# JasonHopeSpace/panda

Measured on AMD Instinct MI355X. Metric: MSM points/s (BN254, 2^24), higher is better.
Workload: dtype u32; 1 GPU; BN254 MSM 2^24 points per GPU, Jacobian output, bases and scalars resident in HBM; curve=bn254, log_points_per_gpu=24, exchange=none

## Files before the change

### panda_amd/csrc/msm_sort.hip

```cpp
#include <algorithm>
#include <atomic>
#include <cmath>

#include "fe29.h"
#include "msm_sort.h"

using namespace panda29;

namespace {

constexpr unsigned SORT_TILE = 8192;
constexpr unsigned MAX_PARTS = 1024;
constexpr unsigned SORT_THREADS = 1024;
constexpr unsigned BS_CHUNK = 8192;

template <class Code>
struct CodeTraits;
template <>
struct CodeTraits<uint16_t> {
    static constexpr u32 ZERO = 0x7fffu;
    static constexpr u32 MAG = 0x7fffu;
    static constexpr int SIGN = 15;
};
template <>
struct CodeTraits<u32> {
    static constexpr u32 ZERO = 0x7fffffffu;
    static constexpr u32 MAG = 0x7fffffffu;
    static constexpr int SIGN = 31;
};

template <int WORDS>
__device__ __forceinline__ void load_words(u32 *dst, const u32 *src)
{
    static_assert(WORDS % 4 == 0, "vector loads");
    const uint4 *s4 = reinterpret_cast<const uint4 *>(src);
#pragma unroll
    for (int i = 0; i < WORDS / 4; i++) {
        uint4 v = s4[i];
        dst[4 * i] = v.x;
        dst[4 * i + 1] = v.y;
        dst[4 * i + 2] = v.z;
        dst[4 * i + 3] = v.w;
    }
}

__device__ __forceinline__ void check_samples(const panda::SampleCheck &sc)
{
    int differs = 0;
    for (unsigned t = threadIdx.x >> 2; t < panda::REG_SAMPLES; t += blockDim.x >> 2) {
        const u64 row = panda::sample_row(t, sc.n);
        for (unsigned k = threadIdx.x & 3u; k < sc.row_words; k += 4) differs |= sc.samples[t * sc.row_words + k] != sc.wire[row * sc.row_words + k];
    }
    differs = __syncthreads_or(differs);
    if (threadIdx.x == 0) {
        *sc.flag_dev = differs ? 1u : 0u;
        if (differs) *sc.flag_host = 1u;
    }
}

struct DigitsBatch {
    unsigned log_n, prefix_bit;
};

template <class Fr, class Code, bool BATCH = false>
__global__ void __launch_bounds__(256) k_digits(const u32 *__restrict__ scalars, Code *__restrict__ dig, u64 n, panda::WindowPlan plan, panda::SampleCheck sc,
                                                DigitsBatch bg)
{
    typedef CodeTraits<Code> CT;
    constexpr int L = Fr::L;
    if (blockIdx.x == 0 && sc.wire) check_samples(sc);
    u64 i = (u64)blockIdx.x * blockDim.x + threadIdx.x;
    if (i >= n) return;
    u32 w[L], s[L + 1];
    load_words<L>(w, scalars + i * L);
    fe_wire_to_canonical<Fr>(s, w);
    s[L] = 0;
    u32 carry = 0;
    const u32 prefix = BATCH ? (u32)(i >> bg.log_n) << bg.prefix_bit : 0u;
    for (unsigned k = 0; k < plan.W; k++) {
        const unsigned c = plan.width[k];
        const u32 half = 1u << (c - 1), full = 1u << c, mask = full - 1;
        unsigned lo = plan.lo[k], m = lo >> 5, sh = lo & 31;
        u32 raw = 0;
        if (m < (unsigned)L) {
            u64 v = s[m] | ((u64)s[m + 1] << 32);
            raw = (u32)(v >> sh) & mask;
        }
        raw += carry;
        u32 code;
        if (raw >= half) {
            u32 mag = full - raw;
            carry = 1;
            code = mag ? ((1u << CT::SIGN) | prefix | (mag - 1)) : CT::ZERO;
        } else {
            carry = 0;
            code = raw ? (prefix | (raw - 1)) : CT::ZERO;
        }
        dig[(u64)k * n + i] = (Code)code;
    }
}

struct DigitsHistGeom {
    unsigned lo_bits, H, tiles;
};

template <class Fr, class Code, bool BATCH = false>
__global__ void __launch_bounds__(1024) k_digits_hist(const u32 *__restrict__ scalars, Code *__restrict__ dig, u32 *__restrict__ tile_hist, u64 n,
                                                     panda::WindowPlan plan, DigitsHistGeom g, panda::SampleCheck sc, DigitsBatch bg)
{
    typedef CodeTraits<Code> CT;
    constexpr int L = Fr::L;
    extern __shared__ u32 hist[];
    if (blockIdx.x == 0 && sc.wire) check_samples(sc);
    const unsigned tile = blockIdx.x, tid = threadIdx.x;
    const unsigned WH = plan.W * g.H, threads = blockDim.x;
    for (unsigned i = tid; i < WH; i += threads) hist[i] = 0;
    __syncthreads();
    const u64 begin = (u64)tile * SORT_TILE, end = begin + SORT_TILE < n ? begin + SORT_TILE : n;
    for (u64 i = begin + tid; i < end; i += threads) {
        u32 w[L], s[L + 1];
        load_words<L>(w, scalars + i * L);
        fe_wire_to_canonical<Fr>(s, w);
        s[L] = 0;
        u32 carry = 0;
        const u32 prefix = BATCH ? (u32)(i >> bg.log_n) << bg.prefix_bit : 0u;
        for (unsigned k = 0; k < plan.W; k++) {
            const unsigned c = plan.width[k];
            const u32 half = 1u << (c - 1), full = 1u << c, mask = full - 1;
            unsigned lo = plan.lo[k], m = lo >> 5, sh = lo & 31;
            u32 raw = 0;
            if (m < (unsigned)L) {
                u64 v = s[m] | ((u64)s[m + 1] << 32);
                raw = (u32)(v >> sh) & mask;
            }
            raw += carry;
            u32 code;
            if (raw >= half) {
                u32 mag = full - raw;
                carry = 1;
                code = mag ? ((1u << CT::SIGN) | prefix | (mag - 1)) : CT::ZERO;
            } else {
                carry = 0;
                code = raw ? (prefix | (raw - 1)) : CT::ZERO;
            }
            dig[(u64)k * n + i] = (Code)code;
            if (code != CT::ZERO) atomicAdd(&hist[k * g.H + ((code & CT::MAG) >> g.lo_bits)], 1u);
        }
    }
    __syncthreads();
    for (unsigned i = tid; i < WH; i += threads) {
        const unsigned k = i / g.H, h = i - k * g.H;
        tile_hist[((u64)k * g.tiles + tile) * g.H + h] = hist[i];
    }
}

template <class Code, class Fn>
__device__ __forceinline__ void for_each_code(const Code *__restrict__ dw, u64 begin, u64 end, Fn f)
{
    constexpr unsigned PER = 16 / sizeof(Code);
    if (reinterpret_cast<uintptr_t>(dw + begin) & 15) {
        for (u64 a = begin + threadIdx.x; a < end; a += blockDim.x) f(a, (u32)dw[a]);
        return;
    }
    for (u64 a = begin + (u64)threadIdx.x * PER; a < end; a += (u64)blockDim.x * PER) {
        const uint4 v = *reinterpret_cast<const uint4 *>(dw + a);
        const u32 wv[4] = {v.x, v.y, v.z, v.w};
#pragma unroll
        for (unsigned j = 0; j < PER; j++) {
            const u32 code = sizeof(Code) == 2 ? (wv[j >> 1] >> (16 * (j & 1))) & 0xffffu : wv[j];
            if (a + j < end) f(a + j, code);
        }
    }
}


struct SortGeom {
    unsigned log_n, lo_bits, H, tiles;
    u32 row0;
};

template <class Code>
__global__ void __launch_bounds__(256) k_part_hist(const Code *__restrict__ dig, u32 *__restrict__ tile_hist, SortGeom g)
{
    typedef CodeTraits<Code> CT;
    __shared__ u32 h[MAX_PARTS];
    const unsigned w = blockIdx.y, tile = blockIdx.x, tid = threadIdx.x;
    for (unsigned i = tid; i < g.H; i += 256) h[i] = 0;
    __syncthreads();
    const u64 n = (u64)1 << g.log_n;
    const Code *dw = dig + ((u64)w << g.log_n);
    const u64 begin = (u64)tile * SORT_TILE, end = begin + SORT_TILE < n ? begin + SORT_TILE : n;
    for_each_code<Code>(dw, begin, end, [&](u64, u32 code) {
        if (code != CT::ZERO) atomicAdd(&h[(code & CT::MAG) >> g.lo_bits], 1u);
    });
    __syncthreads();
    u32 *out = tile_hist + ((u64)w * g.tiles + tile) * g.H;
    for (unsigned i = tid; i < g.H; i += 256) out[i] = h[i];
}

__global__ void __launch_bounds__(1024) k_part_scan_cols(const u32 *__restrict__ tile_hist, u32 *__restrict__ tile_pref, u32 *__restrict__ totals, SortGeom g)
{
    const unsigned w = blockIdx.y, lane = threadIdx.x & 63, h = blockIdx.x * 16 + (threadIdx.x >> 6);
    if (h >= g.H) return;
    const u64 col = (u64)w * g.tiles * g.H + h;
    u32 run = 0;
    for (unsigned t0 = 0; t0 < g.tiles; t0 += 64) {
        const unsigned tile = t0 + lane;
        u32 v = tile < g.tiles ? tile_hist[col + (u64)tile * g.H] : 0;
        u32 inc = v;
        for (unsigned d = 1; d < 64; d <<= 1) {
            u32 up = __shfl_up(inc, d, 64);
            if (lane >= d) inc += up;
        }
        if (tile < g.tiles) tile_pref[col + (u64)tile * g.H] = run + inc - v;
        run += __shfl(inc, 63, 64);
    }
    if (lane == 0) totals[(u64)w * g.H + h] = run;
}

__global__ void __launch_bounds__(1024) k_part_offsets(const u32 *__restrict__ totals, u32 *__restrict__ part_off, SortGeom g)
{
    __shared__ u32 tot[MAX_PARTS];
    const unsigned w = blockIdx.x, t = threadIdx.x;
    const u32 mine = t < g.H ? totals[(u64)w * g.H + t] : 0;
    tot[t] = mine;
    __syncthreads();
    for (unsigned d = 1; d < 1024; d <<= 1) {
        u32 v = (t >= d) ? tot[t - d] : 0;
        __syncthreads();
        tot[t] += v;
        __syncthreads();
    }
    if (t < g.H) part_off[(u64)w * (g.H + 1) + t] = tot[t] - mine;
    if (t == 1023) part_off[(u64)w * (g.H + 1) + g.H] = tot[1023];
}

template <unsigned THREADS = SORT_THREADS>
__device__ __forceinline__ void block_exclusive_scan(u32 *a, unsigned count, u32 *scratch )
{
    const unsigned tid = threadIdx.x;
    const unsigned per = (count + THREADS - 1) / THREADS;
    u32 local = 0;
    for (unsigned j = 0; j < per; j++) {
        unsigned i = tid * per + j;
        if (i < count) local += a[i];
    }
    scratch[tid] = local;
    __syncthreads();
    for (unsigned d = 1; d < THREADS; d <<= 1) {
        u32 v = (tid >= d) ? scratch[tid - d] : 0;
        __syncthreads();
        scratch[tid] += v;
        __syncthreads();
    }
    u32 run = scratch[tid] - local;
    for (unsigned j = 0; j < per; j++) {
        unsigned i = tid * per + j;
        if (i < count) {
            u32 v = a[i];
            a[i] = run;
            run += v;
        }
    }
    __syncthreads();
}

template <class Code, class Word>
__global__ void __launch_bounds__(SORT_THREADS) k_part_scatter(const Code *__restrict__ dig, const u32 *__restrict__ tile_hist, const u32 *__restrict__ tile_pref,
                                                      const u32 *__restrict__ part_off, Word *__restrict__ p1, SortGeom g)
{
    typedef CodeTraits<Code> CT;
    __shared__ u32 lstart[MAX_PARTS];
    __shared__ u32 lcur[MAX_PARTS];
    __shared__ u32 gbase[MAX_PARTS];
    __shared__ Word words[SORT_TILE];
    __shared__ uint16_t parts_of[SORT_TILE];
    __shared__ u32 scratch[SORT_THREADS];
    const unsigned w = blockIdx.y, tile = blockIdx.x, tid = threadIdx.x;
    const u64 row = ((u64)w * g.tiles + tile) * g.H;
    const u32 *po = part_off + (u64)w * (g.H + 1);
    for (unsigned i = tid; i < g.H; i += SORT_THREADS) {
        lstart[i] = tile_hist[row + i];
        lcur[i] = 0;
        gbase[i] = po[i] + tile_pref[row + i];
    }
    __syncthreads();
    const u64 n = (u64)1 << g.log_n;
    const Code *dw = dig + ((u64)w << g.log_n);
    Word *pw = p1 + ((u64)w << g.log_n);
    const u64 begin = (u64)tile * SORT_TILE, end = begin + SORT_TILE < n ? begin + SORT_TILE : n;
    const u32 lo_mask = (1u << g.lo_bits) - 1;
    block_exclusive_scan(lstart, g.H, scratch);
    for_each_code<Code>(dw, begin, end, [&](u64 i, u32 code) {
        if (code == CT::ZERO) return;
        u32 b = code & CT::MAG, h = b >> g.lo_bits;
        u32 slot = lstart[h] + atomicAdd(&lcur[h], 1u);
        words[slot] = ((Word)(b & lo_mask) << (g.log_n + 1)) | (Word)(((code >> CT::SIGN) << g.log_n) | (u32)i);
        parts_of[slot] = (uint16_t)h;
    });
    __syncthreads();
    const u32 total = lstart[g.H - 1] + lcur[g.H - 1];
    for (u32 j = tid; j < total; j += SORT_THREADS) {
        u32 h = parts_of[j];
        pw[gbase[h] + (j - lstart[h])] = words[j];
    }
}

template <class Code>
__global__ void __launch_bounds__(SORT_THREADS) k1_scatter_split(const Code *__restrict__ dig, const u32 *__restrict__ tile_hist, const u32 *__restrict__ tile_pref,
                                                        const u32 *__restrict__ part_off, u32 *__restrict__ p1_lo, unsigned char *__restrict__ p1_hi, SortGeom g,
                                                        unsigned b3)
{
    typedef CodeTraits<Code> CT;
    __shared__ u32 lstart[MAX_PARTS];
    __shared__ u32 lcur[MAX_PARTS];
    __shared__ u32 gbase[MAX_PARTS];
    __shared__ u32 words[SORT_TILE];
    __shared__ unsigned char his[SORT_TILE];
    __shared__ uint16_t parts_of[SORT_TILE];
    __shared__ u32 scratch[SORT_THREADS];
    const unsigned w = blockIdx.y, tile = blockIdx.x, tid = threadIdx.x;
    const u64 row = ((u64)w * g.tiles + tile) * g.H;
    const u32 *po = part_off + (u64)w * (g.H + 1);
    for (unsigned i = tid; i < g.H; i += SORT_THREADS) {
        lstart[i] = tile_hist[row + i];
        lcur[i] = 0;
        gbase[i] = po[i] + tile_pref[row + i];
    }
    __syncthreads();
    const u64 n = (u64)1 << g.log_n;
    const Code *dw = dig + ((u64)w << g.log_n);
    u32 *plo = p1_lo + ((u64)w << g.log_n);
    unsigned char *phi = p1_hi + ((u64)w << g.log_n);
    const u64 begin = (u64)tile * SORT_TILE, end = begin + SORT_TILE < n ? begin + SORT_TILE : n;
    const u32 b3_mask = (1u << b3) - 1, b2_mask = (1u << (g.lo_bits - b3)) - 1;
    block_exclusive_scan(lstart, g.H, scratch);
    for_each_code<Code>(dw, begin, end, [&](u64 i, u32 code) {
        if (code == CT::ZERO) return;
        u32 b = code & CT::MAG, h = b >> g.lo_bits;
        u32 slot = lstart[h] + atomicAdd(&lcur[h], 1u);
        words[slot] = ((b & b3_mask) << (g.log_n + 1)) | ((code >> CT::SIGN) << g.log_n) | (u32)i;
        his[slot] = (unsigned char)((b >> b3) & b2_mask);
        parts_of[slot] = (uint16_t)h;
    });
    __syncthreads();
    const u32 total = lstart[g.H - 1] + lcur[g.H - 1];
    for (u32 j = tid; j < total; j += SORT_THREADS) {
        const u32 h = parts_of[j];
        const u32 dst = gbase[h] + (j - lstart[h]);
        plo[dst] = words[j];
        phi[dst] = his[j];
    }
}

__device__ __forceinline__ void scan128_inclusive(u32 *cnt, u32 *carry )
{
    const unsigned tid = threadIdx.x, lane = tid & 63u;
    u32 v = tid < 128 ? cnt[tid] : 0;
    if (tid < 128) {
        for (unsigned d = 1; d < 64; d <<= 1) {
            const u32 up = __shfl_up(v, d, 64);
            if (lane >= d) v += up;
        }
        if (tid == 63) *carry = v;
    }
    __syncthreads();
    if (tid >= 64 && tid < 128) v += *carry;
    if (tid < 128) cnt[tid] = v;
    __syncthreads();
}

__global__ void __launch_bounds__(SORT_THREADS) k_bucket_sort(const u32 *__restrict__ p1, const u32 *__restrict__ part_off, u32 *__restrict__ off,
                                                     u32 *__restrict__ sorted, SortGeom g, unsigned NB)
{
    __shared__ u32 cnt[128], cur[128], lstart[128], lcur[128], scan_carry;
    __shared__ u32 words[BS_CHUNK];
    __shared__ unsigned char lo_of[BS_CHUNK];
    const unsigned w = blockIdx.y, h = blockIdx.x, tid = threadIdx.x;
    const unsigned L = 1u << g.lo_bits;
    const u32 ps = part_off[(u64)w * (g.H + 1) + h], pe = part_off[(u64)w * (g.H + 1) + h + 1];
    const u32 *pw = p1 + ((u64)w << g.log_n);
    u32 *sw = sorted + ((u64)w << g.log_n);
    const unsigned shift = g.log_n + 1;
    if (tid < 128) cnt[tid] = 0;
    __syncthreads();
    for (u32 j = ps + tid; j < pe; j += SORT_THREADS) atomicAdd(&cnt[pw[j] >> shift], 1u);
    __syncthreads();
    u32 mine = tid < 128 ? cnt[tid] : 0;
    scan128_inclusive(cnt, &scan_carry);
    if (tid < L) {
        u32 start = ps + cnt[tid] - mine;
        cur[tid] = start;
        off[(u64)w * (NB + 1) + ((u64)h << g.lo_bits) + tid] = start;
    }
    if (h == g.H - 1 && tid == 0) off[(u64)w * (NB + 1) + NB] = pe;
    __syncthreads();
    const u32 id_mask = (1u << g.log_n) - 1;
    for (u32 cbeg = ps; cbeg < pe; cbeg += BS_CHUNK) {
        const u32 cend = min(cbeg + BS_CHUNK, pe);
        if (tid < 128) {
            lstart[tid] = 0;
            lcur[tid] = 0;
        }
        __syncthreads();
        for (u32 j = cbeg + tid; j < cend; j += SORT_THREADS) atomicAdd(&lstart[pw[j] >> shift], 1u);
        __syncthreads();
        u32 c0 = tid < 128 ? lstart[tid] : 0;
        scan128_inclusive(lstart, &scan_carry);
        if (tid < 128) {
            lstart[tid] -= c0;
            cnt[tid] = c0;
        }
        __syncthreads();
        for (u32 j = cbeg + tid; j < cend; j += SORT_THREADS) {
            u32 v = pw[j];
            u32 l = v >> shift;
            u32 slot = lstart[l] + atomicAdd(&lcur[l], 1u);
            words[slot] = ((v & id_mask) + g.row0) | (((v >> g.log_n) & 1u) << 31);
            lo_of[slot] = (unsigned char)l;
        }
        __syncthreads();
        for (u32 j = tid; j < cend - cbeg; j += SORT_THREADS) {
            u32 l = lo_of[j];
            sw[cur[l] + (j - lstart[l])] = words[j];
        }
        __syncthreads();
        if (tid < 128) cur[tid] += cnt[tid];
        __syncthreads();
    }
}


struct TabledGeom {
    unsigned log_n, W;
    unsigned b1, b2, b3;
    unsigned H1, H2, S;
    unsigned max_tiles2;
    unsigned Q;
    unsigned row_shift;
    u32 row0;
    unsigned per_window;
    u32 row_mask;
};
__host__ __device__ __forceinline__ unsigned seg_of(const TabledGeom &g, unsigned k, unsigned h1) { return h1 * g.W + k; }

struct SortRange {
    unsigned s_lo, s_hi, q_lo, q_hi;
};

__global__ void __launch_bounds__(SORT_THREADS) k2_seg_tiles(const u32 *__restrict__ part_off, u32 *__restrict__ seg_tile, TabledGeom g)
{
    __shared__ u32 scratch[SORT_THREADS];
    const unsigned tid = threadIdx.x;
    const unsigned per = (g.S + SORT_THREADS - 1) / SORT_THREADS;
    u32 local = 0;
    for (unsigned j = 0; j < per; j++) {
        unsigned s = tid * per + j;
        if (s < g.S) {
            unsigned k = s % g.W, h1 = s / g.W;
            const u32 *po = part_off + (u64)k * (g.H1 + 1);
            local += (po[h1 + 1] - po[h1] + SORT_TILE - 1) / SORT_TILE;
        }
    }
    scratch[tid] = local;
    __syncthreads();
    for (unsigned d = 1; d < SORT_THREADS; d <<= 1) {
        u32 v = (tid >= d) ? scratch[tid - d] : 0;
        __syncthreads();
        scratch[tid] += v;
        __syncthreads();
    }
    u32 run = scratch[tid] - local;
    for (unsigned j = 0; j < per; j++) {
        unsigned s = tid * per + j;
        if (s < g.S) {
            unsigned k = s % g.W, h1 = s / g.W;
            const u32 *po = part_off + (u64)k * (g.H1 + 1);
            seg_tile[s] = run;
            run += (po[h1 + 1] - po[h1] + SORT_TILE - 1) / SORT_TILE;
        }
    }
    if (tid == SORT_THREADS - 1) seg_tile[g.S] = scratch[SORT_THREADS - 1];
}

struct TileRange {
    unsigned s;
    u64 begin, end;
    u64 seg_begin;
};

__device__ __forceinline__ bool locate_tile(TileRange &r, unsigned &tile, unsigned rel, const u32 *seg_tile, const u32 *part_off, const TabledGeom &g, const SortRange &R)
{
    tile = seg_tile[R.s_lo] + rel;
    if (tile >= seg_tile[R.s_hi]) return false;
    unsigned lo = R.s_lo, hi = R.s_hi;
    while (hi - lo > 1) {
        unsigned mid = (lo + hi) >> 1;
        if (seg_tile[mid] <= tile) lo = mid;
        else hi = mid;
    }
    r.s = lo;
    const unsigned k = lo % g.W, h1 = lo / g.W;
    const u32 *po = part_off + (u64)k * (g.H1 + 1);
    r.seg_begin = ((u64)k << g.log_n) + po[h1];
    const u64 seg_end = ((u64)k << g.log_n) + po[h1 + 1];
    r.begin = r.seg_begin + (u64)(tile - seg_tile[lo]) * SORT_TILE;
    r.end = r.begin + SORT_TILE < seg_end ? r.begin + SORT_TILE : seg_end;
    return true;
}

__global__ void __launch_bounds__(256) k2_hist(const unsigned char *__restrict__ p1_hi, const u32 *__restrict__ part_off, const u32 *__restrict__ seg_tile,
                                               u32 *__restrict__ tile_hist, TabledGeom g, SortRange R)
{
    __builtin_amdgcn_s_setprio(3);
    __shared__ u32 h[256];
    const unsigned tid = threadIdx.x;
    unsigned tile;
    TileRange r;
    if (!locate_tile(r, tile, blockIdx.x, seg_tile, part_off, g, R)) return;
    h[tid] = 0;
    __syncthreads();
    const u64 first = r.begin & ~(u64)15;
    for (u64 a = first + (u64)tid * 16; a < r.end; a += 256 * 16) {
        const uint4 v = *reinterpret_cast<const uint4 *>(p1_hi + a);
        const u32 wv[4] = {v.x, v.y, v.z, v.w};
#pragma unroll
        for (int j = 0; j < 16; j++) {
            const u64 i = a + j;
            if (i >= r.begin && i < r.end) atomicAdd(&h[(wv[j >> 2] >> (8 * (j & 3))) & 0xffu], 1u);
        }
    }
    __syncthreads();
    if (tid < g.H2) tile_hist[(u64)tile * g.H2 + tid] = h[tid];
}

__global__ void __launch_bounds__(256) k2_scan_cols(const u32 *__restrict__ tile_hist, u32 *__restrict__ tile_pref, const u32 *__restrict__ seg_tile,
                                                    u32 *__restrict__ totals, TabledGeom g, SortRange R)
{
    __builtin_amdgcn_s_setprio(3);
    const unsigned s = R.s_lo + blockIdx.y, lane = threadIdx.x & 63, h = blockIdx.x * 4 + (threadIdx.x >> 6);
    if (h >= g.H2) return;
    const unsigned t_begin = seg_tile[s], t_end = seg_tile[s + 1];
    u32 run = 0;
    for (unsigned t0 = t_begin; t0 < t_end; t0 += 64) {
        const unsigned tile = t0 + lane;
        u32 v = tile < t_end ? tile_hist[(u64)tile * g.H2 + h] : 0;
        u32 inc = v;
        for (unsigned d = 1; d < 64; d <<= 1) {
            u32 up = __shfl_up(inc, d, 64);
            if (lane >= d) inc += up;
        }
        if (tile < t_end) tile_pref[(u64)tile * g.H2 + h] = run + inc - v;
        run += __shfl(inc, 63, 64);
    }
    if (lane == 0) totals[(u64)s * g.H2 + h] = run;
}

__global__ void __launch_bounds__(256) k2_offsets(const u32 *__restrict__ totals, u32 *__restrict__ sub_off, TabledGeom g, SortRange R)
{
    __builtin_amdgcn_s_setprio(3);
    __shared__ u32 tot[256];
    const unsigned s = R.s_lo + blockIdx.x, t = threadIdx.x;
    const u32 mine = t < g.H2 ? totals[(u64)s * g.H2 + t] : 0;
    tot[t] = mine;
    __syncthreads();
    for (unsigned d = 1; d < 256; d <<= 1) {
        u32 v = (t >= d) ? tot[t - d] : 0;
        __syncthreads();
        tot[t] += v;
        __syncthreads();
    }
    if (t < g.H2) sub_off[(u64)s * (g.H2 + 1) + t] = tot[t] - mine;
    if (t == 255) sub_off[(u64)s * (g.H2 + 1) + g.H2] = tot[255];
}

template <unsigned THREADS>
__global__ void __launch_bounds__(THREADS) k2_scatter(const u32 *__restrict__ p1_lo, const unsigned char *__restrict__ p1_hi, const u32 *__restrict__ part_off,
                                                  const u32 *__restrict__ seg_tile, const u32 *__restrict__ tile_hist, const u32 *__restrict__ tile_pref,
                                                  const u32 *__restrict__ sub_off, u32 *__restrict__ p2, TabledGeom g, SortRange R)
{
    __builtin_amdgcn_s_setprio(3);
    __shared__ u32 lstart[256], lcur[256];
    __shared__ u64 gbase[256];
    __shared__ u32 words[SORT_TILE];
    __shared__ unsigned char parts_of[SORT_TILE];
    __shared__ u32 scratch[THREADS];
    const unsigned tid = threadIdx.x;
    unsigned tile;
    TileRange r;
    if (!locate_tile(r, tile, blockIdx.x, seg_tile, part_off, g, R)) return;
    if (tid < 256) {
        lstart[tid] = tid < g.H2 ? tile_hist[(u64)tile * g.H2 + tid] : 0;
        lcur[tid] = 0;
        if (tid < g.H2) gbase[tid] = r.seg_begin + sub_off[(u64)r.s * (g.H2 + 1) + tid] + tile_pref[(u64)tile * g.H2 + tid];
    }
    __syncthreads();
    block_exclusive_scan<THREADS>(lstart, g.H2, scratch);
    const u64 first = r.begin & ~(u64)15;
    for (u64 a = first + (u64)tid * 16; a < r.end; a += (u64)THREADS * 16) {
        const uint4 kv = *reinterpret_cast<const uint4 *>(p1_hi + a);
        const u32 keys[4] = {kv.x, kv.y, kv.z, kv.w};
        const uint4 *lo4 = reinterpret_cast<const uint4 *>(p1_lo + a);
#pragma unroll
        for (int q = 0; q < 4; q++) {
            const uint4 wv = lo4[q];
            const u32 ws[4] = {wv.x, wv.y, wv.z, wv.w};
#pragma unroll
            for (int j = 0; j < 4; j++) {
                const u64 i = a + 4 * q + j;
                if (i >= r.begin && i < r.end) {
                    const u32 h = (keys[q] >> (8 * j)) & 0xffu;
                    const u32 slot = lstart[h] + atomicAdd(&lcur[h], 1u);
                    words[slot] = ws[j];
                    parts_of[slot] = (unsigned char)h;
                }
            }
        }
    }
    __syncthreads();
    const u32 total = (u32)(r.end - r.begin);
    for (u32 j = tid; j < total; j += THREADS) {
        u32 h = parts_of[j];
        p2[gbase[h] + (j - lstart[h])] = words[j];
    }
}


__device__ __forceinline__ void cell_run(u64 &begin, u32 &len, unsigned k, unsigned h1, unsigned h2, const u32 *part_off, const u32 *sub_off, const TabledGeom &g)
{
    const unsigned s = seg_of(g, k, h1);
    const u32 *so = sub_off + (u64)s * (g.H2 + 1);
    begin = ((u64)k << g.log_n) + part_off[(u64)k * (g.H1 + 1) + h1] + so[h2];
    len = so[h2 + 1] - so[h2];
}

__device__ __forceinline__ unsigned cells_total(const TabledGeom &g) { return g.per_window ? g.W * g.Q : g.Q; }

__global__ void __launch_bounds__(1024) k3_cell_counts(const u32 *__restrict__ sub_off, u32 *__restrict__ cell_cnt, u32 *__restrict__ blk_sum, TabledGeom g, SortRange R)
{
    __builtin_amdgcn_s_setprio(3);
    __shared__ u32 red[16];
    const unsigned blk = R.q_lo / 1024 + blockIdx.x, t = threadIdx.x;
    const unsigned qbits = g.b1 + g.b2;
    u32 sum = 0;
#pragma unroll 1
    for (unsigned q = blk * 1024 + t; q < blk * 1024 + 1024 && q < R.q_hi; q += blockDim.x) {
        const unsigned cell = g.per_window ? q & ((1u << qbits) - 1) : q;
        const unsigned h1 = cell >> g.b2, h2 = cell & (g.H2 - 1);
        const unsigned k_begin = g.per_window ? q >> qbits : 0u, k_end = g.per_window ? k_begin + 1 : g.W;
        u32 total = 0;
#pragma unroll 1
        for (unsigned k = k_begin; k < k_end; k++) {
            const unsigned at = seg_of(g, k, h1) * (g.H2 + 1) + h2;
            total += sub_off[at + 1] - sub_off[at];
        }
        cell_cnt[q] = total;
        sum += total;
    }
    for (unsigned d = 32; d > 0; d >>= 1) sum += __shfl_down(sum, d, 64);
    if ((t & 63) == 0) red[t >> 6] = sum;
    __syncthreads();
    if (t == 0) {
        u32 v = 0;
        for (unsigned i = 0; i < blockDim.x / 64; i++) v += red[i];
        blk_sum[blk] = v;
    }
}

__global__ void __launch_bounds__(1024) k3_cell_offsets(const u32 *__restrict__ cell_cnt, const u32 *__restrict__ blk_sum, u32 *__restrict__ cell_off, TabledGeom g, SortRange R)
{
    __builtin_amdgcn_s_setprio(3);
    __shared__ u32 red[1024];
    __shared__ u32 sc[1024];
    const unsigned blk = R.q_lo / 1024 + blockIdx.x, t = threadIdx.x, T = blockDim.x, per = 1024 / T;
    u32 v = 0;
    for (unsigned b = t; b < blk; b += T) v += blk_sum[b];
    red[t] = v;
    const unsigned q0 = blk * 1024 + t * per;
    u32 local = 0;
    for (unsigned j = 0; j < per; j++) local += q0 + j < R.q_hi ? cell_cnt[q0 + j] : 0;
    sc[t] = local;
    __syncthreads();
    for (unsigned s = T >> 1; s > 0; s >>= 1) {
        if (t < s) red[t] += red[t + s];
        __syncthreads();
    }
    for (unsigned d = 1; d < T; d <<= 1) {
        u32 u = (t >= d) ? sc[t - d] : 0;
        __syncthreads();
        sc[t] += u;
        __syncthreads();
    }
    u32 run = red[0] + sc[t] - local;
    for (unsigned j = 0; j < per; j++) {
        const unsigned q = q0 + j;
        if (q < R.q_hi) {
            cell_off[q] = run;
            run += cell_cnt[q];
            if (q == R.q_hi - 1) cell_off[R.q_hi] = run;
        }
    }
}

constexpr unsigned K3_THREADS = 1024;
constexpr unsigned K3_PER = 16;
constexpr unsigned K3_CAP = K3_THREADS * K3_PER;
constexpr unsigned K3_PER_WIDE = 32;

#ifdef PANDA_K3_STAMPS
__device__ unsigned long long g_k3_stamps[1024 * 8];
#define K3_STAMP(n)                                                                                                          \
    do {                                                                                                                     \
        if (threadIdx.x == 0 && (cell & 15u) == 0 && (cell >> 4) < 1024) g_k3_stamps[(cell >> 4) * 8 + (n)] = __builtin_amdgcn_s_memrealtime(); \
    } while (0)
#else
#define K3_STAMP(n)
#endif

template <unsigned PER, unsigned THREADS = K3_THREADS, bool BATCH = false>
__global__ void __launch_bounds__(THREADS) k3_merge(const u32 *__restrict__ p2, const u32 *__restrict__ part_off, const u32 *__restrict__ sub_off,
                                              const u32 *__restrict__ cell_off, u32 *__restrict__ off, u32 *__restrict__ sorted, TabledGeom g, unsigned NB, SortRange R)
{
    __shared__ u32 cnt[128], cur[128], scan_carry;
    constexpr unsigned IMG = THREADS * K3_PER;
    __shared__ u32 outbuf[IMG];
    __shared__ u64 rbegin[64];
    __shared__ u32 rlen[64];
    __shared__ u32 vstart[65];
    const unsigned tid = threadIdx.x;
    const unsigned cell = R.q_lo + blockIdx.x;
    const unsigned k0 = g.per_window ? cell / g.Q : 0u, q = g.per_window ? cell % g.Q : cell;
    const unsigned nruns = g.per_window ? 1u : g.W;
    const unsigned h1 = q / g.H2, h2 = q % g.H2;
    const unsigned L = 1u << g.b3;
    K3_STAMP(0);
    const u32 out_rel = cell_off[cell] - (g.per_window ? cell_off[k0 * g.Q] : 0u);
    const bool closes_part = !g.per_window && cell + 1 == R.q_hi && q + 1 < g.Q;
    u32 *sw = sorted + ((u64)k0 << g.log_n);
    u32 *ow = off + (u64)k0 * (NB + 1);
    if (tid < nruns) {
        u64 b;
        u32 len;
        cell_run(b, len, k0 + tid, h1, h2, part_off, sub_off, g);
        rbegin[tid] = b;
        rlen[tid] = len;
    }
    if (tid < 128) cnt[tid] = 0;
    __syncthreads();
    if (tid == 0) {
        u32 run = 0;
        for (unsigned k = 0; k < nruns; k++) {
            vstart[k] = run;
            run += rlen[k];
        }
        vstart[nruns] = run;
    }
    __syncthreads();
    K3_STAMP(1);
    const u32 N = vstart[nruns];
    const unsigned shift = g.log_n + 1;
    const u32 id_mask = (1u << g.log_n) - 1;
    auto window_of = [&](u32 p) -> unsigned {
        unsigned k = 0;
        for (unsigned j = 1; j < nruns; j++) k += p >= vstart[j] ? 1u : 0u;
        return k;
    };
    const unsigned table_shift = g.per_window ? 32u : g.row_shift;
    auto final_word = [&](u32 v, unsigned k) -> u32 {
        const u32 id = BATCH ? v & id_mask & g.row_mask : v & id_mask;
        return (id + g.row0 + (table_shift < 32 ? (k << table_shift) : 0u)) | (((v >> g.log_n) & 1u) << 31);
    };

    if (closes_part && tid == 0) ow[(u64)(q + 1) << g.b3] = out_rel + N;
    if (N == 0) {
        if (tid < L) ow[((u64)q << g.b3) + tid] = out_rel;
        if (q == g.Q - 1 && tid == 0) ow[NB] = out_rel;
        return;
    }
    if (N <= THREADS * PER) {
        u32 word[PER];
        u32 where[PER];
        unsigned k = 0;
#pragma unroll
        for (unsigned j = 0; j < PER; j++) {
            const u32 p = min(tid + j * THREADS, N - 1);
            while (p >= vstart[k + 1]) k++;
            where[j] = k;
            word[j] = p2[rbegin[k] + (p - vstart[k])];
        }
        K3_STAMP(2);
#ifdef PANDA_K3_STAMPS
        __builtin_amdgcn_s_waitcnt(0x0f70);
        K3_STAMP(3);
#endif
#pragma unroll
        for (unsigned j = 0; j < PER; j++) {
            const u32 p = tid + j * THREADS;
            if (p < N) {
                const u32 v = word[j];
                word[j] = final_word(v, where[j]);
                const u32 b = v >> shift;
                where[j] = (atomicAdd(&cnt[b], 1u) << 7) | b;
            }
        }
        K3_STAMP(4);
        __syncthreads();
        K3_STAMP(5);
        u32 mine = tid < 128 ? cnt[tid] : 0;
        scan128_inclusive(cnt, &scan_carry);
        if (tid < L) {
            const u32 start = cnt[tid] - mine;
            cur[tid] = start;
            ow[((u64)q << g.b3) + tid] = out_rel + start;
        }
        if (q == g.Q - 1 && tid == 0) ow[NB] = out_rel + N;
        __syncthreads();
#pragma unroll
        for (unsigned j = 0; j < PER; j++) {
            const u32 p = tid + j * THREADS;
            if (p < N) where[j] = cur[where[j] & 127u] + (where[j] >> 7);
        }
#pragma unroll 1
        for (u32 base = 0; base < N; base += IMG) {
            if (base) __syncthreads();
#pragma unroll
            for (unsigned j = 0; j < PER; j++) {
                const u32 p = tid + j * THREADS;
                if (p < N && where[j] - base < IMG) outbuf[where[j] - base] = word[j];
            }
            __syncthreads();
            const u32 len = min(N - base, IMG);
            for (u32 p = tid; p < len; p += THREADS) sw[out_rel + base + p] = outbuf[p];
        }
        K3_STAMP(7);
        return;
    }

    for (u32 p = tid; p < N; p += THREADS) {
        const unsigned k = window_of(p);
        atomicAdd(&cnt[p2[rbegin[k] + (p - vstart[k])] >> shift], 1u);
    }
    __syncthreads();
    u32 mine = tid < 128 ? cnt[tid] : 0;
    for (unsigned d = 1; d < 128; d <<= 1) {
        u32 v = (tid < 128 && tid >= d) ? cnt[tid - d] : 0;
        __syncthreads();
        if (tid < 128) cnt[tid] += v;
        __syncthreads();
    }
    if (tid < L) {
        u32 start = out_rel + cnt[tid] - mine;
        cur[tid] = start;
        ow[((u64)q << g.b3) + tid] = start;
    }
    if (q == g.Q - 1 && tid == 0) ow[NB] = out_rel + N;
    __syncthreads();
    for (u32 p = tid; p < N; p += THREADS) {
        const unsigned k = window_of(p);
        const u32 v = p2[rbegin[k] + (p - vstart[k])];
        sw[atomicAdd(&cur[v >> shift], 1u)] = final_word(v, k);
    }
    K3_STAMP(6);
}

template <unsigned THREADS>
__global__ void __launch_bounds__(THREADS) k3_merge_small(const u32 *__restrict__ p2, const u32 *__restrict__ part_off, const u32 *__restrict__ sub_off,
                                                 const u32 *__restrict__ cell_off, u32 *__restrict__ off, u32 *__restrict__ sorted, TabledGeom g, unsigned NB, SortRange R)
{
    __builtin_amdgcn_s_setprio(3);
    constexpr bool STAGED = THREADS >= 1024;
    __shared__ u32 cnt[128], cur[128], scan_carry;
    __shared__ u32 outbuf[STAGED ? K3_CAP : 1];
    __shared__ u32 rbegin_lo[64], vstart[65];
    const unsigned tid = threadIdx.x;
    const unsigned q = R.q_lo + blockIdx.x;
    const unsigned h1 = q / g.H2, h2 = q % g.H2;
    const unsigned L = 1u << g.b3;
    const u32 out_rel = cell_off[q];
    if (tid < g.W) {
        const unsigned at = seg_of(g, tid, h1) * (g.H2 + 1) + h2;
        const u32 so = sub_off[at];
        rbegin_lo[tid] = part_off[tid * (g.H1 + 1) + h1] + so;
        vstart[tid + 1] = sub_off[at + 1] - so;
    }
    if (tid < 128) cnt[tid] = 0;
    __syncthreads();
    if (tid == 0) {
        u32 run = 0;
        for (unsigned k = 0; k < g.W; k++) {
            const u32 len = vstart[k + 1];
            vstart[k] = run;
            run += len;
        }
        vstart[g.W] = run;
    }
    __syncthreads();
    const u32 N = vstart[g.W];
    const unsigned shift = g.log_n + 1;
    if (q + 1 == R.q_hi && q + 1 < g.Q && tid == 0) off[(u64)(q + 1) << g.b3] = out_rel + N;
    if (N == 0) {
        if (tid < L) off[((u64)q << g.b3) + tid] = out_rel;
        if (q == g.Q - 1 && tid == 0) off[NB] = out_rel;
        return;
    }
    unsigned k = 0;
#pragma unroll 1
    for (u32 p = tid; p < N; p += THREADS) {
        while (p >= vstart[k + 1]) k++;
        atomicAdd(&cnt[p2[((u64)k << g.log_n) + rbegin_lo[k] + (p - vstart[k])] >> shift], 1u);
// ... 435 lines not shown
```

Baseline: 983.7 million points/s.

## Use wave-shuffle block scans and restructure digit extraction and partition scatters

```diff
diff --git a/panda_amd/csrc/msm_sort.hip b/panda_amd/csrc/msm_sort.hip
--- a/panda_amd/csrc/msm_sort.hip
+++ b/panda_amd/csrc/msm_sort.hip
@@ -62,30 +62,18 @@
     unsigned log_n, prefix_bit;
 };
 
-template <class Fr, class Code, bool BATCH = false>
-__global__ void __launch_bounds__(256) k_digits(const u32 *__restrict__ scalars, Code *__restrict__ dig, u64 n, panda::WindowPlan plan, panda::SampleCheck sc,
-                                                DigitsBatch bg)
-{
-    typedef CodeTraits<Code> CT;
-    constexpr int L = Fr::L;
-    if (blockIdx.x == 0 && sc.wire) check_samples(sc);
-    u64 i = (u64)blockIdx.x * blockDim.x + threadIdx.x;
-    if (i >= n) return;
-    u32 w[L], s[L + 1];
-    load_words<L>(w, scalars + i * L);
-    fe_wire_to_canonical<Fr>(s, w);
-    s[L] = 0;
+__device__ __forceinline__ void stage_plan(u32 *wlo, const panda::WindowPlan &plan)
+{
+    for (unsigned k = threadIdx.x; k < plan.W; k += blockDim.x) wlo[k] = plan.lo[k] | ((u32)plan.width[k] << 16);
+}
+
+template <int L, class CT, class Fn>
+__device__ __forceinline__ void for_each_digit(const u32 *s, const u32 *wlo, unsigned W, u32 prefix, Fn f)
+{
     u32 carry = 0;
-    const u32 prefix = BATCH ? (u32)(i >> bg.log_n) << bg.prefix_bit : 0u;
-    for (unsigned k = 0; k < plan.W; k++) {
-        const unsigned c = plan.width[k];
-        const u32 half = 1u << (c - 1), full = 1u << c, mask = full - 1;
-        unsigned lo = plan.lo[k], m = lo >> 5, sh = lo & 31;
-        u32 raw = 0;
-        if (m < (unsigned)L) {
-            u64 v = s[m] | ((u64)s[m + 1] << 32);
-            raw = (u32)(v >> sh) & mask;
-        }
+    unsigned k = 0;
+    auto digit = [&](u32 raw, unsigned c) {
+        const u32 half = 1u << (c - 1), full = 1u << c;
         raw += carry;
         u32 code;
         if (raw >= half) {
@@ -96,8 +84,40 @@
             carry = 0;
             code = raw ? (prefix | (raw - 1)) : CT::ZERO;
         }
-        dig[(u64)k * n + i] = (Code)code;
-    }
+        f(k, code);
+    };
+#pragma unroll
+    for (int m = 0; m < L; m++) {
+        const u64 v = s[m] | ((u64)s[m + 1] << 32);
+        while (k < W) {
+            const u32 e = __builtin_amdgcn_readfirstlane(wlo[k]);
+            const unsigned lo = e & 0xffffu, c = e >> 16;
+            if ((lo >> 5) != (unsigned)m) break;
+            digit((u32)(v >> (lo & 31)) & ((1u << c) - 1), c);
+            k++;
+        }
+    }
+    for (; k < W; k++) digit(0, __builtin_amdgcn_readfirstlane(wlo[k]) >> 16);
+}
+
+template <class Fr, class Code, bool BATCH = false>
+__global__ void __launch_bounds__(256) k_digits(const u32 *__restrict__ scalars, Code *__restrict__ dig, u64 n, panda::WindowPlan plan, panda::SampleCheck sc,
+                                                DigitsBatch bg)
+{
+    typedef CodeTraits<Code> CT;
+    constexpr int L = Fr::L;
+    __shared__ u32 wlo[panda::MAX_WINDOWS];
+    if (blockIdx.x == 0 && sc.wire) check_samples(sc);
+    stage_plan(wlo, plan);
+    __syncthreads();
+    u64 i = (u64)blockIdx.x * blockDim.x + threadIdx.x;
+    if (i >= n) return;
+    u32 w[L], s[L + 1];
+    load_words<L>(w, scalars + i * L);
+    fe_wire_to_canonical<Fr>(s, w);
+    s[L] = 0;
+    const u32 prefix = BATCH ? (u32)(i >> bg.log_n) << bg.prefix_bit : 0u;
+    for_each_digit<L, CT>(s, wlo, plan.W, prefix, [&](unsigned k, u32 code) { dig[(u64)k * n + i] = (Code)code; });
 }
 
 struct DigitsHistGeom {
@@ -111,41 +131,26 @@
     typedef CodeTraits<Code> CT;
     constexpr int L = Fr::L;
     extern __shared__ u32 hist[];
+    __shared__ u32 wlo[panda::MAX_WINDOWS];
     if (blockIdx.x == 0 && sc.wire) check_samples(sc);
     const unsigned tile = blockIdx.x, tid = threadIdx.x;
     const unsigned WH = plan.W * g.H, threads = blockDim.x;
     for (unsigned i = tid; i < WH; i += threads) hist[i] = 0;
+    stage_plan(wlo, plan);
     __syncthreads();
     const u64 begin = (u64)tile * SORT_TILE, end = begin + SORT_TILE < n ? begin + SORT_TILE : n;
+    u32 w[L];
+    if (begin + tid < end) load_words<L>(w, scalars + (begin + tid) * L);
     for (u64 i = begin + tid; i < end; i += threads) {
-        u32 w[L], s[L + 1];
-        load_words<L>(w, scalars + i * L);
+        u32 s[L + 1];
         fe_wire_to_canonical<Fr>(s, w);
+        if (i + threads < end) load_words<L>(w, scalars + (i + threads) * L);
         s[L] = 0;
-        u32 carry = 0;
         const u32 prefix = BATCH ? (u32)(i >> bg.log_n) << bg.prefix_bit : 0u;
-        for (unsigned k = 0; k < plan.W; k++) {
-            const unsigned c = plan.width[k];
-            const u32 half = 1u << (c - 1), full = 1u << c, mask = full - 1;
-            unsigned lo = plan.lo[k], m = lo >> 5, sh = lo & 31;
-            u32 raw = 0;
-            if (m < (unsigned)L) {
-                u64 v = s[m] | ((u64)s[m + 1] << 32);
-                raw = (u32)(v >> sh) & mask;
-            }
-            raw += carry;
-            u32 code;
-            if (raw >= half) {
-                u32 mag = full - raw;
-                carry = 1;
-                code = mag ? ((1u << CT::SIGN) | prefix | (mag - 1)) : CT::ZERO;
-            } else {
-                carry = 0;
-                code = raw ? (prefix | (raw - 1)) : CT::ZERO;
-            }
+        for_each_digit<L, CT>(s, wlo, plan.W, prefix, [&](unsigned k, u32 code) {
             dig[(u64)k * n + i] = (Code)code;
             if (code != CT::ZERO) atomicAdd(&hist[k * g.H + ((code & CT::MAG) >> g.lo_bits)], 1u);
-        }
+        });
     }
     __syncthreads();
     for (unsigned i = tid; i < WH; i += threads) {
@@ -218,92 +223,115 @@
     if (lane == 0) totals[(u64)w * g.H + h] = run;
 }
 
+__device__ __forceinline__ u32 block_inclusive_scan(u32 v, u32 *wsum)
+{
+    const unsigned lane = threadIdx.x & 63u, wave = threadIdx.x >> 6;
+    for (unsigned d = 1; d < 64; d <<= 1) {
+        const u32 up = __shfl_up(v, d, 64);
+        if (lane >= d) v += up;
+    }
+    if (lane == 63) wsum[wave] = v;
+    __syncthreads();
+    for (unsigned w = 0; w < wave; w++) v += wsum[w];
+    return v;
+}
+
 __global__ void __launch_bounds__(1024) k_part_offsets(const u32 *__restrict__ totals, u32 *__restrict__ part_off, SortGeom g)
 {
-    __shared__ u32 tot[MAX_PARTS];
+    __shared__ u32 wsum[16];
     const unsigned w = blockIdx.x, t = threadIdx.x;
     const u32 mine = t < g.H ? totals[(u64)w * g.H + t] : 0;
-    tot[t] = mine;
-    __syncthreads();
-    for (unsigned d = 1; d < 1024; d <<= 1) {
-        u32 v = (t >= d) ? tot[t - d] : 0;
-        __syncthreads();
-        tot[t] += v;
-        __syncthreads();
-    }
-    if (t < g.H) part_off[(u64)w * (g.H + 1) + t] = tot[t] - mine;
-    if (t == 1023) part_off[(u64)w * (g.H + 1) + g.H] = tot[1023];
-}
-
-template <unsigned THREADS = SORT_THREADS>
-__device__ __forceinline__ void block_exclusive_scan(u32 *a, unsigned count, u32 *scratch )
-{
-    const unsigned tid = threadIdx.x;
-    const unsigned per = (count + THREADS - 1) / THREADS;
-    u32 local = 0;
-    for (unsigned j = 0; j < per; j++) {
-        unsigned i = tid * per + j;
-        if (i < count) local += a[i];
-    }
-    scratch[tid] = local;
-    __syncthreads();
-    for (unsigned d = 1; d < THREADS; d <<= 1) {
-        u32 v = (tid >= d) ? scratch[tid - d] : 0;
-        __syncthreads();
-        scratch[tid] += v;
-        __syncthreads();
-    }
-    u32 run = scratch[tid] - local;
-    for (unsigned j = 0; j < per; j++) {
-        unsigned i = tid * per + j;
-        if (i < count) {
-            u32 v = a[i];
-            a[i] = run;
-            run += v;
-        }
-    }
-    __syncthreads();
-}
+    const u32 inc = block_inclusive_scan(mine, wsum);
+    if (t < g.H) part_off[(u64)w * (g.H + 1) + t] = inc - mine;
+    if (t == 1023) part_off[(u64)w * (g.H + 1) + g.H] = inc;
+}
+
+template <class Code, unsigned THREADS>
+struct TileCodes {
+    static constexpr unsigned PER = 16 / sizeof(Code), LOADS = SORT_TILE / (THREADS * PER);
+    static_assert(LOADS * THREADS * PER == SORT_TILE, "whole loads");
+    uint4 v[LOADS];
+    bool vec;
+    __device__ __forceinline__ void load(const Code *__restrict__ dw, u64 begin, u64 end)
+    {
+        vec = !(reinterpret_cast<uintptr_t>(dw + begin) & 15);
+        if (!vec) return;
+#pragma unroll
+        for (unsigned q = 0; q < LOADS; q++) {
+            const u64 a = begin + ((u64)q * THREADS + threadIdx.x) * PER;
+            v[q] = a < end ? *reinterpret_cast<const uint4 *>(dw + a) : uint4{0, 0, 0, 0};
+        }
+    }
+    __device__ __forceinline__ u32 code(unsigned q, unsigned j) const
+    {
+        const u32 wv[4] = {v[q].x, v[q].y, v[q].z, v[q].w};
+        return sizeof(Code) == 2 ? (wv[j >> 1] >> (16 * (j & 1))) & 0xffffu : wv[j];
+    }
+    template <class Rank, class Place>
+    __device__ __forceinline__ void rank_and_place(const Code *__restrict__ dw, u64 begin, u64 end, Rank rank, Place place) const
+    {
+        if (!vec) {
+            for_each_code<Code>(dw, begin, end, [&](u64 i, u32 c) { place(i, c, rank(i, c)); });
+            return;
+        }
+        u32 slot[LOADS * PER];
+#pragma unroll
+        for (unsigned q = 0; q < LOADS; q++) {
+            const u64 a = begin + ((u64)q * THREADS + threadIdx.x) * PER;
+#pragma unroll
+            for (unsigned j = 0; j < PER; j++)
+                if (a + j < end) slot[q * PER + j] = rank(a + j, code(q, j));
+        }
+#pragma unroll
+        for (unsigned q = 0; q < LOADS; q++) {
+            const u64 a = begin + ((u64)q * THREADS + threadIdx.x) * PER;
+#pragma unroll
+            for (unsigned j = 0; j < PER; j++)
+                if (a + j < end) place(a + j, code(q, j), slot[q * PER + j]);
+        }
+    }
+};
 
 template <class Code, class Word>
 __global__ void __launch_bounds__(SORT_THREADS) k_part_scatter(const Code *__restrict__ dig, const u32 *__restrict__ tile_hist, const u32 *__restrict__ tile_pref,
                                                       const u32 *__restrict__ part_off, Word *__restrict__ p1, SortGeom g)
 {
     typedef CodeTraits<Code> CT;
-    __shared__ u32 lstart[MAX_PARTS];
+    static_assert(MAX_PARTS <= SORT_THREADS, "a partition counter per thread");
     __shared__ u32 lcur[MAX_PARTS];
-    __shared__ u32 gbase[MAX_PARTS];
+    __shared__ u32 delta[MAX_PARTS];
     __shared__ Word words[SORT_TILE];
     __shared__ uint16_t parts_of[SORT_TILE];
-    __shared__ u32 scratch[SORT_THREADS];
+    __shared__ u32 wsum[SORT_THREADS / 64];
     const unsigned w = blockIdx.y, tile = blockIdx.x, tid = threadIdx.x;
     const u64 row = ((u64)w * g.tiles + tile) * g.H;
     const u32 *po = part_off + (u64)w * (g.H + 1);
-    for (unsigned i = tid; i < g.H; i += SORT_THREADS) {
-        lstart[i] = tile_hist[row + i];
-        lcur[i] = 0;
-        gbase[i] = po[i] + tile_pref[row + i];
-    }
-    __syncthreads();
     const u64 n = (u64)1 << g.log_n;
     const Code *dw = dig + ((u64)w << g.log_n);
     Word *pw = p1 + ((u64)w << g.log_n);
     const u64 begin = (u64)tile * SORT_TILE, end = begin + SORT_TILE < n ? begin + SORT_TILE : n;
     const u32 lo_mask = (1u << g.lo_bits) - 1;
-    block_exclusive_scan(lstart, g.H, scratch);
-    for_each_code<Code>(dw, begin, end, [&](u64 i, u32 code) {
-        if (code == CT::ZERO) return;
-        u32 b = code & CT::MAG, h = b >> g.lo_bits;
-        u32 slot = lstart[h] + atomicAdd(&lcur[h], 1u);
-        words[slot] = ((Word)(b & lo_mask) << (g.log_n + 1)) | (Word)(((code >> CT::SIGN) << g.log_n) | (u32)i);
-        parts_of[slot] = (uint16_t)h;
-    });
-    __syncthreads();
-    const u32 total = lstart[g.H - 1] + lcur[g.H - 1];
-    for (u32 j = tid; j < total; j += SORT_THREADS) {
-        u32 h = parts_of[j];
-        pw[gbase[h] + (j - lstart[h])] = words[j];
-    }
+    TileCodes<Code, SORT_THREADS> codes;
+    codes.load(dw, begin, end);
+    const u32 count = tid < g.H ? tile_hist[row + tid] : 0;
+    const u32 gbase = tid < g.H ? po[tid] + tile_pref[row + tid] : 0;
+    const u32 lstart = block_inclusive_scan(count, wsum) - count;
+    if (tid < g.H) {
+        lcur[tid] = lstart;
+        delta[tid] = gbase - lstart;
+    }
+    __syncthreads();
+    codes.rank_and_place(
+        dw, begin, end, [&](u64, u32 code) -> u32 { return code == CT::ZERO ? 0u : atomicAdd(&lcur[(code & CT::MAG) >> g.lo_bits], 1u); },
+        [&](u64 i, u32 code, u32 slot) {
+            if (code == CT::ZERO) return;
+            u32 b = code & CT::MAG, h = b >> g.lo_bits;
+            words[slot] = ((Word)(b & lo_mask) << (g.log_n + 1)) | (Word)(((code >> CT::SIGN) << g.log_n) | (u32)i);
+            parts_of[slot] = (uint16_t)h;
+        });
+    __syncthreads();
+    const u32 total = lcur[g.H - 1];
+    for (u32 j = tid; j < total; j += SORT_THREADS) pw[delta[parts_of[j]] + j] = words[j];
 }
 
 template <class Code>
@@ -312,44 +340,59 @@
                                                         unsigned b3)
 {
     typedef CodeTraits<Code> CT;
-    __shared__ u32 lstart[MAX_PARTS];
+    static_assert(MAX_PARTS <= SORT_THREADS, "a partition counter per thread");
     __shared__ u32 lcur[MAX_PARTS];
-    __shared__ u32 gbase[MAX_PARTS];
+    __shared__ u32 delta[MAX_PARTS];
     __shared__ u32 words[SORT_TILE];
-    __shared__ unsigned char his[SORT_TILE];
-    __shared__ uint16_t parts_of[SORT_TILE];
-    __shared__ u32 scratch[SORT_THREADS];
-    const unsigned w = blockIdx.y, tile = blockIdx.x, tid = threadIdx.x;
+    __shared__ u32 meta[SORT_TILE];
+    __shared__ u32 wsum[SORT_THREADS / 64];
+    const unsigned w = blockIdx.y, tile = blockIdx.x, tid = threadIdx.x, lane = tid & 63u;
     const u64 row = ((u64)w * g.tiles + tile) * g.H;
     const u32 *po = part_off + (u64)w * (g.H + 1);
-    for (unsigned i = tid; i < g.H; i += SORT_THREADS) {
-        lstart[i] = tile_hist[row + i];
-        lcur[i] = 0;
-        gbase[i] = po[i] + tile_pref[row + i];
-    }
-    __syncthreads();
     const u64 n = (u64)1 << g.log_n;
     const Code *dw = dig + ((u64)w << g.log_n);
     u32 *plo = p1_lo + ((u64)w << g.log_n);
     unsigned char *phi = p1_hi + ((u64)w << g.log_n);
     const u64 begin = (u64)tile * SORT_TILE, end = begin + SORT_TILE < n ? begin + SORT_TILE : n;
     const u32 b3_mask = (1u << b3) - 1, b2_mask = (1u << (g.lo_bits - b3)) - 1;
-    block_exclusive_scan(lstart, g.H, scratch);
-    for_each_code<Code>(dw, begin, end, [&](u64 i, u32 code) {
-        if (code == CT::ZERO) return;
-        u32 b = code & CT::MAG, h = b >> g.lo_bits;
-        u32 slot = lstart[h] + atomicAdd(&lcur[h], 1u);
-        words[slot] = ((b & b3_mask) << (g.log_n + 1)) | ((code >> CT::SIGN) << g.log_n) | (u32)i;
-        his[slot] = (unsigned char)((b >> b3) & b2_mask);
-        parts_of[slot] = (uint16_t)h;
-    });
-    __syncthreads();
-    const u32 total = lstart[g.H - 1] + lcur[g.H - 1];
-    for (u32 j = tid; j < total; j += SORT_THREADS) {
-        const u32 h = parts_of[j];
-        const u32 dst = gbase[h] + (j - lstart[h]);
-        plo[dst] = words[j];
-        phi[dst] = his[j];
+    TileCodes<Code, SORT_THREADS> codes;
+    codes.load(dw, begin, end);
+    const u32 count = tid < g.H ? tile_hist[row + tid] : 0;
+    const u32 gbase = tid < g.H ? po[tid] + tile_pref[row + tid] : 0;
+    const u32 lstart = block_inclusive_scan(count, wsum) - count;
+    if (tid < g.H) {
+        lcur[tid] = lstart;
+        delta[tid] = gbase - lstart;
+    }
+    __syncthreads();
+    codes.rank_and_place(
+        dw, begin, end, [&](u64, u32 code) -> u32 { return code == CT::ZERO ? 0u : atomicAdd(&lcur[(code & CT::MAG) >> g.lo_bits], 1u); },
+        [&](u64 i, u32 code, u32 slot) {
+            if (code == CT::ZERO) return;
+            u32 b = code & CT::MAG, h = b >> g.lo_bits;
+            words[slot] = ((b & b3_mask) << (g.log_n + 1)) | ((code >> CT::SIGN) << g.log_n) | (u32)i;
+            meta[slot] = (h << 8) | ((b >> b3) & b2_mask);
+        });
+    __syncthreads();
+    const u32 total = lcur[g.H - 1];
+    for (u32 base = 0; base < total; base += SORT_THREADS) {
+        const u32 j = base + tid;
+        const bool valid = j < total;
+        const u32 m = valid ? meta[j] : ~0u;
+        const u32 h = m >> 8;
+        u32 dst = 0;
+        if (valid) {
+            dst = delta[h] + j;
+            plo[dst] = words[j];
+        }
+        const u32 m1 = __shfl_down(m, 1, 64), m2 = __shfl_down(m, 2, 64), m3 = __shfl_down(m, 3, 64);
+        const bool lead = valid && lane <= 60 && !(reinterpret_cast<uintptr_t>(phi + dst) & 3) && (m1 >> 8) == h && (m2 >> 8) == h && (m3 >> 8) == h;
+        const u64 leaders = __ballot(lead);
+        const bool covered = (((leaders << 1) | (leaders << 2) | (leaders << 3)) >> lane) & 1;
+        if (lead)
+            *reinterpret_cast<u32 *>(phi + dst) = (m & 0xffu) | ((m1 & 0xffu) << 8) | ((m2 & 0xffu) << 16) | (m3 << 24);
+        else if (valid && !covered)
+            phi[dst] = (unsigned char)m;
     }
 }
 
@@ -450,7 +493,7 @@
 
 __global__ void __launch_bounds__(SORT_THREADS) k2_seg_tiles(const u32 *__restrict__ part_off, u32 *__restrict__ seg_tile, TabledGeom g)
 {
-    __shared__ u32 scratch[SORT_THREADS];
+    __shared__ u32 wsum[SORT_THREADS / 64];
     const unsigned tid = threadIdx.x;
     const unsigned per = (g.S + SORT_THREADS - 1) / SORT_THREADS;
     u32 local = 0;
@@ -462,15 +505,8 @@
             local += (po[h1 + 1] - po[h1] + SORT_TILE - 1) / SORT_TILE;
         }
     }
-    scratch[tid] = local;
-    __syncthreads();
-    for (unsigned d = 1; d < SORT_THREADS; d <<= 1) {
-        u32 v = (tid >= d) ? scratch[tid - d] : 0;
-        __syncthreads();
-        scratch[tid] += v;
-        __syncthreads();
-    }
-    u32 run = scratch[tid] - local;
+    const u32 inc = block_inclusive_scan(local, wsum);
+    u32 run = inc - local;
     for (unsigned j = 0; j < per; j++) {
         unsigned s = tid * per + j;
         if (s < g.S) {
@@ -480,7 +516,7 @@
             run += (po[h1 + 1] - po[h1] + SORT_TILE - 1) / SORT_TILE;
         }
     }
-    if (tid == SORT_THREADS - 1) seg_tile[g.S] = scratch[SORT_THREADS - 1];
+    if (tid == SORT_THREADS - 1) seg_tile[g.S] = inc;
 }
 
 struct TileRange {
@@ -559,19 +595,12 @@
 __global__ void __launch_bounds__(256) k2_offsets(const u32 *__restrict__ totals, u32 *__restrict__ sub_off, TabledGeom g, SortRange R)
 {
     __builtin_amdgcn_s_setprio(3);
-    __shared__ u32 tot[256];
+    __shared__ u32 wsum[4];
     const unsigned s = R.s_lo + blockIdx.x, t = threadIdx.x;
     const u32 mine = t < g.H2 ? totals[(u64)s * g.H2 + t] : 0;
-    tot[t] = mine;
-    __syncthreads();
-    for (unsigned d = 1; d < 256; d <<= 1) {
-        u32 v = (t >= d) ? tot[t - d] : 0;
-        __syncthreads();
-        tot[t] += v;
-        __syncthreads();
-    }
-    if (t < g.H2) sub_off[(u64)s * (g.H2 + 1) + t] = tot[t] - mine;
-    if (t == 255) sub_off[(u64)s * (g.H2 + 1) + g.H2] = tot[255];
+    const u32 inc = block_inclusive_scan(mine, wsum);
+    if (t < g.H2) sub_off[(u64)s * (g.H2 + 1) + t] = inc - mine;
+    if (t == 255) sub_off[(u64)s * (g.H2 + 1) + g.H2] = inc;
 }
 
 template <unsigned THREADS>
@@ -580,49 +609,58 @@
                                                   const u32 *__restrict__ sub_off, u32 *__restrict__ p2, TabledGeom g, SortRange R)
 {
     __builtin_amdgcn_s_setprio(3);
-    __shared__ u32 lstart[256], lcur[256];
-    __shared__ u64 gbase[256];
+    __shared__ u32 lcur[256];
+    __shared__ u32 delta[256];
     __shared__ u32 words[SORT_TILE];
     __shared__ unsigned char parts_of[SORT_TILE];
-    __shared__ u32 scratch[THREADS];
+    __shared__ u32 wsum[THREADS / 64];
+    static_assert(THREADS >= 256, "a sub-partition counter per thread");
     const unsigned tid = threadIdx.x;
     unsigned tile;
     TileRange r;
     if (!locate_tile(r, tile, blockIdx.x, seg_tile, part_off, g, R)) return;
-    if (tid < 256) {
-        lstart[tid] = tid < g.H2 ? tile_hist[(u64)tile * g.H2 + tid] : 0;
-        lcur[tid] = 0;
-        if (tid < g.H2) gbase[tid] = r.seg_begin + sub_off[(u64)r.s * (g.H2 + 1) + tid] + tile_pref[(u64)tile * g.H2 + tid];
-    }
-    __syncthreads();
-    block_exclusive_scan<THREADS>(lstart, g.H2, scratch);
-    const u64 first = r.begin & ~(u64)15;
-    for (u64 a = first + (u64)tid * 16; a < r.end; a += (u64)THREADS * 16) {
-        const uint4 kv = *reinterpret_cast<const uint4 *>(p1_hi + a);
-        const u32 keys[4] = {kv.x, kv.y, kv.z, kv.w};
-        const uint4 *lo4 = reinterpret_cast<const uint4 *>(p1_lo + a);
-#pragma unroll
-        for (int q = 0; q < 4; q++) {
-            const uint4 wv = lo4[q];
-            const u32 ws[4] = {wv.x, wv.y, wv.z, wv.w};
-#pragma unroll
-            for (int j = 0; j < 4; j++) {
-                const u64 i = a + 4 * q + j;
-                if (i >= r.begin && i < r.end) {
-                    const u32 h = (keys[q] >> (8 * j)) & 0xffu;
-                    const u32 slot = lstart[h] + atomicAdd(&lcur[h], 1u);
-                    words[slot] = ws[j];
-                    parts_of[slot] = (unsigned char)h;
-                }
+    const u64 first = r.begin & ~(u64)7, a0 = first + (u64)tid * 8;
+    uint2 kv{0, 0};
+    uint4 w0{0, 0, 0, 0}, w1{0, 0, 0, 0};
+    if (a0 < r.end) {
+        kv = *reinterpret_cast<const uint2 *>(p1_hi + a0);
+        w0 = *reinterpret_cast<const uint4 *>(p1_lo + a0);
+        w1 = *reinterpret_cast<const uint4 *>(p1_lo + a0 + 4);
+    }
+    const u32 count = tid < g.H2 ? tile_hist[(u64)tile * g.H2 + tid] : 0;
+    const u32 gbase = tid < g.H2 ? (u32)r.seg_begin + sub_off[(u64)r.s * (g.H2 + 1) + tid] + tile_pref[(u64)tile * g.H2 + tid] : 0;
+    const u32 lstart = block_inclusive_scan(count, wsum) - count;
+    if (tid < g.H2) {
+        lcur[tid] = lstart;
+        delta[tid] = gbase - lstart;
+    }
+    __syncthreads();
+    for (u64 a = a0; a < r.end; a += (u64)THREADS * 8) {
+        if (a != a0) {
+            kv = *reinterpret_cast<const uint2 *>(p1_hi + a);
+            w0 = *reinterpret_cast<const uint4 *>(p1_lo + a);
+            w1 = *reinterpret_cast<const uint4 *>(p1_lo + a + 4);
+        }
+        const u32 keys[2] = {kv.x, kv.y};
+        const u32 ws[8] = {w0.x, w0.y, w0.z, w0.w, w1.x, w1.y, w1.z, w1.w};
+        u32 slot[8];
+#pragma unroll
+        for (int j = 0; j < 8; j++) {
+            const u64 i = a + j;
+            if (i >= r.begin && i < r.end) slot[j] = atomicAdd(&lcur[(keys[j >> 2] >> (8 * (j & 3))) & 0xffu], 1u);
+        }
+#pragma unroll
+        for (int j = 0; j < 8; j++) {
+            const u64 i = a + j;
+            if (i >= r.begin && i < r.end) {
+                words[slot[j]] = ws[j];
+                parts_of[slot[j]] = (unsigned char)((keys[j >> 2] >> (8 * (j & 3))) & 0xffu);
             }
         }
     }
     __syncthreads();
     const u32 total = (u32)(r.end - r.begin);
-    for (u32 j = tid; j < total; j += THREADS) {
-        u32 h = parts_of[j];
-        p2[gbase[h] + (j - lstart[h])] = words[j];
-    }
+    for (u32 j = tid; j < total; j += THREADS) p2[delta[parts_of[j]] + j] = words[j];
 }
 
 
@@ -670,28 +708,17 @@
 __global__ void __launch_bounds__(1024) k3_cell_offsets(const u32 *__restrict__ cell_cnt, const u32 *__restrict__ blk_sum, u32 *__restrict__ cell_off, TabledGeom g, SortRange R)
 {
     __builtin_amdgcn_s_setprio(3);
-    __shared__ u32 red[1024];
-    __shared__ u32 sc[1024];
+    __shared__ u32 wsum[16], wsum_before[16], before;
     const unsigned blk = R.q_lo / 1024 + blockIdx.x, t = threadIdx.x, T = blockDim.x, per = 1024 / T;
     u32 v = 0;
     for (unsigned b = t; b < blk; b += T) v += blk_sum[b];
-    red[t] = v;
     const unsigned q0 = blk * 1024 + t * per;
     u32 local = 0;
     for (unsigned j = 0; j < per; j++) local += q0 + j < R.q_hi ? cell_cnt[q0 + j] : 0;
-    sc[t] = local;
-    __syncthreads();
-    for (unsigned s = T >> 1; s > 0; s >>= 1) {
-        if (t < s) red[t] += red[t + s];
-        __syncthreads();
-    }
-    for (unsigned d = 1; d < T; d <<= 1) {
-        u32 u = (t >= d) ? sc[t - d] : 0;
-        __syncthreads();
-        sc[t] += u;
-        __syncthreads();
-    }
-    u32 run = red[0] + sc[t] - local;
+    v = block_inclusive_scan(v, wsum_before);
+    if (t == T - 1) before = v;
+    const u32 inc = block_inclusive_scan(local, wsum);
+    u32 run = before + inc - local;
     for (unsigned j = 0; j < per; j++) {
         const unsigned q = q0 + j;
         if (q < R.q_hi) {
@@ -725,7 +752,6 @@
     constexpr unsigned IMG = THREADS * K3_PER;
     __shared__ u32 outbuf[IMG];
     __shared__ u64 rbegin[64];
-    __shared__ u32 rlen[64];
     __shared__ u32 vstart[65];
     const unsigned tid = threadIdx.x;
     const unsigned cell = R.q_lo + blockIdx.x;
@@ -738,23 +764,22 @@
     const bool closes_part = !g.per_window && cell + 1 == R.q_hi && q + 1 < g.Q;
     u32 *sw = sorted + ((u64)k0 << g.log_n);
     u32 *ow = off + (u64)k0 * (NB + 1);
-    if (tid < nruns) {
-        u64 b;
-        u32 len;
-        cell_run(b, len, k0 + tid, h1, h2, part_off, sub_off, g);
-        rbegin[tid] = b;
-        rlen[tid] = len;
+    if (tid < 64) {
+        u64 b = 0;
+        u32 len = 0;
+        if (tid < nruns) {
+            cell_run(b, len, k0 + tid, h1, h2, part_off, sub_off, g);
+            rbegin[tid] = b;
+        }
+        u32 inc = len;
+        for (unsigned d = 1; d < 64; d <<= 1) {
+            const u32 up = __shfl_up(inc, d, 64);
+            if (tid >= d) inc += up;
+        }
+        if (tid < nruns) vstart[tid] = inc - len;
+        if (tid == nruns - 1) vstart[nruns] = inc;
     }
     if (tid < 128) cnt[tid] = 0;
-    __syncthreads();
-    if (tid == 0) {
-        u32 run = 0;
-        for (unsigned k = 0; k < nruns; k++) {
-            vstart[k] = run;
-            run += rlen[k];
-        }
-        vstart[nruns] = run;
-    }
     __syncthreads();
     K3_STAMP(1);
     const u32 N = vstart[nruns];
```

Result: faster. 1.001 billion points/s (median of 6 runs) (+1.8%).
